# dot-comma-hyphen/oaxaca-blinder-rs

Measured on AMD Instinct MI355X. Metric: bootstrap replicates/sec on 1M-row×20-pred panel at 1/2/4/8 MI355X, higher is better.
Workload: dtype f64

## Files before the change

oaxaca-blinder-rs_amd/csrc/ob_engine.hip:

```cpp
#include <hip/hip_runtime.h>

#include <algorithm>
#include <cmath>
#include <cstdio>
#include <cstdlib>
#include <cstring>
#include <map>
#include <mutex>
#include <vector>

#include "ob_device.hpp"
#include "ob_engine.hpp"
#include "ob_hip.hpp"
#include "ob_heckman.hpp"
#include "ob_options.hpp"
#include "ob_spec.h"

typedef double ob_d4 __attribute__((ext_vector_type(4)));

namespace {

constexpr int kBlock = 256;
constexpr int kImgRow = 64;
constexpr int kImgWords = (OB_TILE_ROWS / 4) * kImgRow;
// ... 102 lines not shown
  const uint32_t c4 = c >> 12;
  ob_bitstream s = {q << 12, rep, c2, OB_TAG_L1K + rl, k0, k1, 0u, 0u, 0u, 0u, 0u};
  if (q < c4) return ky_walk(s, L, OB_KY_TABLES - 1, goff, glist);
  const uint32_t i = q - c4, nd = (uint32_t)__builtin_popcount((c >> 7) & 31u);
  if (i < nd) return ky_walk(s, L, (int)ob_l1_digit_log(c, i) - OB_KY_MIN_LOG, goff, glist);
  return ob_bs_popcount(s, c & 127u);
}

template <int DIAG>
__global__ __launch_bounds__(kBlock) __attribute__((amdgpu_waves_per_eu(8, 8))) void ob_level1_kernel(uint32_t n0, uint32_t n1, uint32_t tiles0,
                                                           uint32_t first_rep, uint32_t stride,
                                                           uint32_t key0, uint32_t key1, uint32_t* m1,
                                                           const ob_ky_tables ky_g) {
  extern __shared__ __attribute__((aligned(16))) uint32_t l1s[];
  __shared__ uint32_t s_rej, s_tail, s_acc;
  __shared__ KyLds kyl;
  const uint32_t g = blockIdx.y, rl = blockIdx.x, rep = first_rep + rl, tid = threadIdx.x;
  const uint32_t n = g ? n1 : n0;
  if (n == 0) return;
  if constexpr (!(DIAG & 4)) ky_stage(kyl, ky_g, tid);
  if constexpr ((DIAG & 16) != 0) {
    __syncthreads();
    if (tid == 0 && kyl.hlist[7] == 0xFFFFu) m1[0] = 0u;
    return;
  }
  const uint32_t T = (n + OB_TILE_ROWS - 1) >> OB_TILE_SHIFT, D = l1_depth(T), J = l1_top_levels(T);
  const uint32_t tail = n - (T - 1) * OB_TILE_ROWS;
  const bool small = l1_small(T), partial = tail < OB_TILE_ROWS;
  uint32_t* buf[2] = {l1s, l1s + l1_buf0_words(T)};
  uint32_t* top[2] = {buf[1] + (l1_sub_tiles(T) + 1) / 2, buf[1] + (l1_sub_tiles(T) + 1) / 2 + kL1TopWords};
  uint32_t* mt = l1s + 256u + 128u;
  uint32_t* mcol = m1 + (size_t)rl * stride + (g ? tiles0 : 0u);
  const uint32_t tail_owner = ((T - 1) >> 1) & (kBlock - 1);
  if (small && tid < T) mt[tid] = 0;
  uint32_t todo = n;
  for (uint32_t round = 0;; ++round) {
    if (tid == 0) {
      if (J) top[0][0] = todo;
      else buf[D & 1][0] = todo;
      s_rej = 0;
      s_tail = 0;
      s_acc = 0;
    }
    __syncthreads();
    uint32_t rej = 0;
    auto emit = [&](uint32_t t, uint32_t c) {
      if constexpr ((DIAG & 8) != 0) return;
      if (partial && t == T - 1) s_tail = c;
      else if (round == 0) mcol[t] = c;
      else if (c) mcol[t] += c;
    };
    auto level = [&](uint32_t l, uint32_t ll, uint32_t kb, uint32_t nodes, const uint32_t* cur, uint32_t* nxt) {
      const uint32_t span = 1u << (D - l - 1);
      const uint32_t nnext = (T + span - 1) / span;
      const uint32_t rl = (round << 5) + l;
      if (ll < 8) {
        const uint32_t sh = 8 - ll, k = tid >> sh, j = tid & ((1u << sh) - 1);
        if (j == 0 && k < nodes) nxt[2 * k] = 0;
        __syncthreads();
        uint32_t c = 0;
        if (k < nodes) {
          c = cur[k];
          uint32_t left = 0;
          if constexpr (DIAG & 1) left = j == 0 ? c >> 1 : 0u;
          else if (c < OB_KY_MIN_C) left = l1_split_words(j, 1u << sh, c, rep, ((kb + k) << 1) | g, rl, key0, key1);
          else
            for (uint32_t q = j, ns = ob_l1_items(c); q < ns; q += 1u << sh)
              left += l1_split_item(q, c, rep, ((kb + k) << 1) | g, rl, key0, key1, kyl, ky_g.off, ky_g.list);
          if (left) atomicAdd(&nxt[2 * k], left);
        }
        __syncthreads();
        if (j == 0 && k < nodes) {
          const uint32_t right = c - nxt[2 * k];
          if (2 * (kb + k) + 1 < nnext) nxt[2 * k + 1] = right;
          else rej += right;
        }
        __syncthreads();
      } else {
        const bool to_m1 = l + 1 == D && !small;
        for (uint32_t k = tid; k < nodes; k += kBlock) {
          const uint32_t c = cur[k], kg = kb + k;
          uint32_t left = 0;
          if constexpr (DIAG & 1) left = c >> 1;
          else if ((DIAG & 32) && c < 128u) left = c >> 1;
          else if (c < OB_KY_MIN_C) left = l1_split_words(0, 1, c, rep, (kg << 1) | g, rl, key0, key1);
          else
            for (uint32_t q = 0, ns = ob_l1_items(c); q < ns; ++q)
              left += l1_split_item(q, c, rep, (kg << 1) | g, rl, key0, key1, kyl, ky_g.off, ky_g.list);
          const uint32_t right = c - left;
          if (to_m1) {
            emit(2 * kg, left);
            if (2 * kg + 1 < T) emit(2 * kg + 1, right);
            else rej += right;
          } else {
            nxt[2 * k] = left;
            if (2 * kg + 1 < nnext) nxt[2 * k + 1] = right;
            else rej += right;
          }
        }
        __syncthreads();
      }
    };
    for (uint32_t l = 0; l < J; ++l) {
      const uint32_t span2 = 2u << (D - l - 1);
      level(l, l, 0, (T + span2 - 1) / span2, top[l & 1], top[(l + 1) & 1]);
    }
    const uint32_t nsub = J ? (T + (1u << (D - J)) - 1) >> (D - J) : 1u;
    for (uint32_t K = 0; K < nsub; ++K) {
      if (J) {
        if (tid == 0) buf[(D - J) & 1][0] = top[J & 1][K];
        __syncthreads();
      }
      for (uint32_t l = J; l < D; ++l) {
        const uint32_t ll = l - J, kb = K << ll, span2 = 2u << (D - l - 1);
        const uint32_t nodes = min(1u << ll, (T + span2 - 1) / span2 - kb);
        level(l, ll, kb, nodes, buf[(D - l) & 1], buf[(D - l - 1) & 1]);
      }
    }
    if (small) {
      const uint32_t* tl = buf[0];
      if (tid < T) {
        if (partial && tid == T - 1) s_tail = tl[tid];
        else mt[tid] += tl[tid];
      }
      __syncthreads();
    }
    if (partial && tid < 64) {
      const uint32_t c = s_tail;
      uint32_t acc = 0;
      for (uint32_t q = tid; 16 * q < c; q += 64) {
        const ob_u32x4 u = ob_philox(q, rep, g, OB_TAG_L1S + round, key0, key1);
        const uint32_t wd[4] = {u.x, u.y, u.z, u.w};
        const uint32_t m = min(16u, c - 16 * q);
#pragma unroll
        for (uint32_t i = 0; i < 16; ++i) acc += (i < m && ((wd[i >> 2] >> (8 * (i & 3))) & 0xFFu) < tail) ? 1u : 0u;
      }
      if (acc) atomicAdd(&s_acc, acc);
    }
    __syncthreads();
    if (partial) {
      const uint32_t a = s_acc;
      if (tid == 0) rej += s_tail - a;
      if (small) {
        if (tid == 0) mt[T - 1] += a;
      } else if (tid == tail_owner) {
        if (round == 0) mcol[T - 1] = a;
        else if (a) mcol[T - 1] += a;
      }
    }
    if (rej) atomicAdd(&s_rej, rej);
    __syncthreads();
    todo = s_rej;
    __syncthreads();
    if (todo <= OB_L1_DIRECT) break;
    if constexpr ((DIAG & 2) != 0) {
      todo = 0;
      break;
    }
  }
  __syncthreads();
  for (uint32_t r = tid; r < todo; r += kBlock) {
    const uint32_t thresh = (0u - n) % n;
    uint64_t x;
    for (uint32_t j = 0;; ++j) {
      const ob_u32x4 u = ob_philox(r, rep, g, OB_TAG_L1D + (j >> 2), key0, key1);
      const uint32_t wd[4] = {u.x, u.y, u.z, u.w};
      x = (uint64_t)wd[j & 3] * n;
      if ((uint32_t)x >= thresh) break;
    }
    const uint32_t t = (uint32_t)(x >> 32) >> OB_TILE_SHIFT;
    if (small) atomicAdd(&mt[t], 1u);
    else atomicAdd(&mcol[t], 1u);
  }
  if (small) {
    __syncthreads();
    if (tid < T) mcol[tid] = mt[tid];
  }
}

struct Work {
  uint32_t rb, cg, chunk, g, t0, t1, n, rep0;
  const double* X;
  int64_t ld;
};

__device__ __forceinline__ Work map_work(const GramArgs& a) {
  const uint32_t nwg = gridDim.x, bid = blockIdx.x;
  const uint32_t xcd = bid & 7u, slot = bid >> 3, q8 = nwg >> 3, r8 = nwg & 7u;
  const uint32_t wi = (xcd < r8 ? xcd * (q8 + 1) : r8 * (q8 + 1) + (xcd - r8) * q8) + slot;
  Work w;
  w.rb = wi % a.nb_rep;
  const uint32_t tq = wi / a.nb_rep;
  w.cg = tq % (uint32_t)a.n_cg;
  w.chunk = tq / (uint32_t)a.n_cg;
  w.g = a.chunks[w.chunk * 3];
  w.t0 = a.chunks[w.chunk * 3 + 1];
  w.t1 = a.chunks[w.chunk * 3 + 2];
  w.X = w.g ? a.gcols1 : a.gcols0;
  w.ld = w.g ? a.ld1 : a.ld0;
  w.n = w.g ? a.n1 : a.n0;
  w.rep0 = w.rb * 64;
  return w;
}

__device__ __forceinline__ void lds_barrier() { asm volatile("s_waitcnt lgkmcnt(0)\n\ts_barrier" ::: "memory"); }

template <int CB>
__device__ __forceinline__ void pair_offsets(const GramArgs& a, int cb0, int lane, int (&offa)[CB], int (&offb)[CB]) {
#pragma unroll
  for (int c = 0; c < CB; ++c) {
    const int e = (cb0 + c) * 16 + (lane & 15);
    int pa = 0, pb = 0;
    if (e < a.e) {
      int rem = e;
      while (rem >= a.k1 - pa) {
        rem -= a.k1 - pa;
        ++pa;
      }
      pb = pa + rem;
    }
    offa[c] = pa * kColStride + (lane >> 4) * 16 + (pa & 31);
    offb[c] = pb * kColStride + (lane >> 4) * 16 + (pb & 31);
  }
}

__device__ __forceinline__ void stage_dma(const GramArgs& a, const Work& w, uint32_t xt_byte_off, size_t gbase,
                                          int wave, int w_lo, int nw, int lane,
                                          __attribute__((address_space(3))) unsigned char* lds3) {
  const int ncl = a.k1 - a.c_first;
  const uint32_t bytes = (uint32_t)ncl * kColStride * 8;
  const char* src = reinterpret_cast<const char*>(w.X + (gbase >> 6) * (size_t)ncl * kColStride);
  const uint32_t dst = xt_byte_off + (uint32_t)a.c_first * kColStride * 8;
  for (uint32_t t = wave - w_lo; t * 1024 < bytes; t += nw)
    if (t * 1024 + lane * 16 < bytes)
      __builtin_amdgcn_global_load_lds(src + t * 1024 + lane * 16,
                                       (__attribute__((address_space(3))) void*)(lds3 + dst + t * 1024), 16, 0, 0);
}

static_assert(OB_TILE_ROWS == 256u, "full-tile draws are bytes");
__device__ __forceinline__ bool full_tile(const Work& w, uint32_t tile) {
  return w.n - tile * OB_TILE_ROWS >= OB_TILE_ROWS;
}

__device__ __forceinline__ void add_draw(uint32_t* img, uint32_t r, uint32_t lr) {
  atomicAdd(&img[(lr >> 2) * kImgRow + r], 1u << ((lr & 3u) * 8u));
}

template <int H>
__device__ __forceinline__ uint32_t sdwa_add_half(uint32_t base, uint32_t a) {
  uint32_t r;
  if constexpr (H == 0)
    asm("v_add_u32_sdwa %0, %1, %2 dst_sel:DWORD dst_unused:UNUSED_PAD src0_sel:DWORD src1_sel:WORD_0" : "=v"(r) : "v"(base), "v"(a));
  else
    asm("v_add_u32_sdwa %0, %1, %2 dst_sel:DWORD dst_unused:UNUSED_PAD src0_sel:DWORD src1_sel:WORD_1" : "=v"(r) : "v"(base), "v"(a));
  return r;
}

template <int B>
__device__ __forceinline__ uint32_t sdwa_shl_byte(uint32_t m, uint32_t one) {
  uint32_t r;
  if constexpr (B == 0)
    asm("v_lshlrev_b32_sdwa %0, %1, %2 dst_sel:DWORD dst_unused:UNUSED_PAD src0_sel:BYTE_0 src1_sel:DWORD" : "=v"(r) : "v"(m), "v"(one));
  else if constexpr (B == 1)
    asm("v_lshlrev_b32_sdwa %0, %1, %2 dst_sel:DWORD dst_unused:UNUSED_PAD src0_sel:BYTE_1 src1_sel:DWORD" : "=v"(r) : "v"(m), "v"(one));
  else if constexpr (B == 2)
    asm("v_lshlrev_b32_sdwa %0, %1, %2 dst_sel:DWORD dst_unused:UNUSED_PAD src0_sel:BYTE_2 src1_sel:DWORD" : "=v"(r) : "v"(m), "v"(one));
  else
    asm("v_lshlrev_b32_sdwa %0, %1, %2 dst_sel:DWORD dst_unused:UNUSED_PAD src0_sel:BYTE_3 src1_sel:DWORD" : "=v"(r) : "v"(m), "v"(one));
  return r;
}

template <int B>
__device__ __forceinline__ void add_draw_byte(uint32_t* img, uint32_t rep_off, uint32_t a, uint32_t m, uint32_t one) {
  atomicAdd(reinterpret_cast<uint32_t*>(reinterpret_cast<char*>(img) + sdwa_add_half<(B >> 1)>(rep_off, a)),
            sdwa_shl_byte<B>(m, one));
}

#ifndef OB_CNT_PERM
#define OB_CNT_PERM 1
#endif
template <int B>
__device__ __forceinline__ void add_draw_perm(uint32_t* img, uint32_t rep_off, uint32_t q, uint32_t m, uint32_t one) {
  const uint32_t addr = __builtin_amdgcn_perm(q, rep_off, 0x0C0C0000u | ((4u + B) << 8));
  atomicAdd(reinterpret_cast<uint32_t*>(reinterpret_cast<char*>(img) + addr), sdwa_shl_byte<B>(m, one));
}

__device__ __forceinline__ void add_draws_word(uint32_t* img, uint32_t rep_off, uint32_t w, uint32_t one) {
  const uint32_t m = (w << 3) & 0x18181818u;
  if (OB_CNT_PERM) {
    const uint32_t q = (w >> 2) & 0x3F3F3F3Fu;
    add_draw_perm<0>(img, rep_off, q, m, one);
    add_draw_perm<1>(img, rep_off, q, m, one);
    add_draw_perm<2>(img, rep_off, q, m, one);
    add_draw_perm<3>(img, rep_off, q, m, one);
    return;
  }
  const uint32_t lo = (w << 6) & 0x3F003F00u, hi = (w >> 2) & 0x3F003F00u;
  add_draw_byte<0>(img, rep_off, lo, m, one);
  add_draw_byte<1>(img, rep_off, hi, m, one);
  add_draw_byte<2>(img, rep_off, lo, m, one);
  add_draw_byte<3>(img, rep_off, hi, m, one);
}

__device__ __forceinline__ void level2_draws(const GramArgs& a, const Work& w, uint32_t tile, uint32_t* cnt,
                                             const uint32_t* mc, const uint32_t* cum, int k, int nparts, int wv,
                                             int nw, int lane) {
  const uint32_t S = min(OB_TILE_ROWS, w.n - tile * OB_TILE_ROWS);
  const bool full = S == OB_TILE_ROWS;
  const int r_lo = 64 * wv / nw, r_hi = 64 * (wv + 1) / nw, nr = r_hi - r_lo;
  if (nr <= 0) return;
  const uint32_t c_lo = cum[r_lo], C = cum[r_hi] - c_lo;
  const uint32_t f_lo = c_lo + C * (uint32_t)k / (uint32_t)nparts;
  const uint32_t f_hi = c_lo + C * (uint32_t)(k + 1) / (uint32_t)nparts;
  const uint32_t bnd = lane < nr ? cum[r_lo + 1 + lane] : 0xFFFFFFFFu;
  const uint32_t c2 = (tile << 1) | w.g;
  const uint32_t rep0 = a.first_rep + w.rep0;
  const uint32_t one = 1u;
  int rr = r_lo;
  for (uint32_t f0 = f_lo; f0 < f_hi; f0 += 64) {
    while (rr < r_hi - 1 && (uint32_t)__builtin_amdgcn_readlane(bnd, rr - r_lo) <= f0) ++rr;
    const uint32_t f = f0 + lane;
    int r = rr;
    uint32_t base = rr > r_lo ? (uint32_t)__builtin_amdgcn_readlane(bnd, rr - r_lo - 1) : c_lo;
    for (int i = rr; i < r_hi - 1; ++i) {
      const uint32_t b = (uint32_t)__builtin_amdgcn_readlane(bnd, i - r_lo);
      if (b > f0 + 63) break;
      if (f >= b) {
        r = i + 1;
        base = b;
      }
    }
    if (f < f_hi) {
      const uint32_t pp = f - base;
      ob_u32x4 u;
      if (a.diag & 64)
        u = ob_u32x4{pp * 0x9E3779B9u ^ r, pp * 0x85EBCA6Bu ^ c2, pp * 0xC2B2AE35u, pp ^ 0x27D4EB2Fu};
      else
        u = ob_philox_x3(pp, rep0 + r, c2, OB_TAG_L2, a.key0, a.key1);
      if (full && (a.diag & 32)) {
        if ((u.x ^ u.y ^ u.z ^ u.w) == 0x5EED5EEDu) cnt[r] = 1u;
      } else if (full) {
        const uint32_t wd[4] = {u.x, u.y, u.z, u.w};
#pragma unroll
        for (int i = 0; i < 4; ++i) add_draws_word(cnt, (uint32_t)r * 4u, wd[i], one);
      } else {
        add_draw(cnt, (uint32_t)r, ob_mulhi64(u.x, u.y, S));
        if (2 * pp + 1 < mc[r]) add_draw(cnt, (uint32_t)r, ob_mulhi64(u.z, u.w, S));
      }
    }
  }
  if (full && k == nparts - 1 && lane < nr) {
    const int r = r_lo + lane;
    const uint32_t m = mc[r], nd = m & 15u;
    if (nd) {
      const ob_u32x4 u = ob_philox_x3(m >> 4, rep0 + r, c2, OB_TAG_L2, a.key0, a.key1);
      const uint32_t wd[4] = {u.x, u.y, u.z, u.w};
#pragma unroll
      for (uint32_t d = 0; d < 15; ++d)
        if (d < nd) add_draw(cnt, (uint32_t)r, (wd[d >> 2] >> (8 * (d & 3))) & 0xFFu);
    }
  }
}

constexpr uint32_t kCallMapCap = 2048;

__device__ __forceinline__ void level2_map_draws(const GramArgs& a, const Work& w, uint32_t tile, uint32_t* cnt,
                                                 const uint32_t* mc, const uint32_t* cmap, uint32_t C,
                                                 uint32_t cmin, int wv, int lane) {
  const uint32_t nwin = (C + 63u) >> 6;
  const uint32_t c2 = (tile << 1) | w.g;
  const uint32_t rep0 = a.first_rep + w.rep0;
  const uint32_t one = 1u;
  for (uint32_t win = (uint32_t)wv; win <= nwin; win += 4) {
    if (win < nwin) {
      const uint32_t f = win * 64u + (uint32_t)lane;
      if (f < C) {
        uint32_t r = (uint32_t)lane, pp = win;
        if (win >= cmin) {
          const uint32_t e = cmap[f - cmin * 64u];
          r = e & 63u;
          pp = e >> 6;
        }
        ob_u32x4 u;
        if (a.diag & 64)
          u = ob_u32x4{pp * 0x9E3779B9u ^ r, pp * 0x85EBCA6Bu ^ c2, pp * 0xC2B2AE35u, pp ^ 0x27D4EB2Fu};
        else
          u = ob_philox_x3(pp, rep0 + r, c2, OB_TAG_L2, a.key0, a.key1);
        if (a.diag & 32) {
          if ((u.x ^ u.y ^ u.z ^ u.w) == 0x5EED5EEDu) cnt[r] = 1u;
        } else {
          const uint32_t wd[4] = {u.x, u.y, u.z, u.w};
#pragma unroll
          for (int i = 0; i < 4; ++i) add_draws_word(cnt, r * 4u, wd[i], one);
        }
      }
    } else {
      const uint32_t m = mc[lane], nd = m & 15u;
      if (nd) {
        const ob_u32x4 u = ob_philox_x3(m >> 4, rep0 + (uint32_t)lane, c2, OB_TAG_L2, a.key0, a.key1);
        const uint32_t wd[4] = {u.x, u.y, u.z, u.w};
#pragma unroll
        for (uint32_t d = 0; d < 15; ++d)
          if (d < nd) add_draw(cnt, (uint32_t)lane, (wd[d >> 2] >> (8 * (d & 3))) & 0xFFu);
      }
    }
  }
}

#ifndef OB_CNT_NT
#define OB_CNT_NT 0
#endif
template <bool I8>
__device__ __forceinline__ void check_store_counts(const GramArgs& a, uint32_t* cnt, uint32_t* lsum, int my,
                                                   uint32_t tt, uint32_t rb, uint32_t ns) {
  const int r = my & 63, part = my >> 6;
  uint32_t* col = cnt + part * 16 * kImgRow + r;
  uint32_t v[16];
  uint32_t sum = 0, hib = 0;
#pragma unroll
  for (int i = 0; i < 16; ++i) {
    v[i] = col[i * kImgRow];
    sum = __builtin_amdgcn_sad_u8(v[i], 0u, sum);
    hib |= v[i] & 0x80808080u;
  }
  if (I8 && hib && !(a.diag & 1632)) atomicOr(a.flags, 2u);
  if ((uint32_t)part < ns && !(a.diag & 512)) {
    if constexpr (I8) {
      uint4* out = reinterpret_cast<uint4*>(const_cast<uint32_t*>(a.counts)) + ((size_t)tt * a.nb_rep + rb) * 1024 +
                   part * 256 + (r >> 4) * 64 + (r & 15);
#pragma unroll
      for (int q = 0; q < 4; ++q) {
        if (OB_CNT_NT) {
          typedef unsigned int u32x4_t __attribute__((ext_vector_type(4)));
          const u32x4_t u4 = {v[4 * q], v[4 * q + 1], v[4 * q + 2], v[4 * q + 3]};
          __builtin_nontemporal_store(u4, reinterpret_cast<u32x4_t*>(out + q * 16));
        } else {
          out[q * 16] = make_uint4(v[4 * q], v[4 * q + 1], v[4 * q + 2], v[4 * q + 3]);
        }
      }
    } else {
      uint32_t* out = const_cast<uint32_t*>(a.counts) + ((size_t)tt * a.nb_rep + rb) * 4 * kCimgWords +
                      part * kCimgWords + r * kCimgStride;
#pragma unroll
      for (int i = 0; i < 16; ++i) out[i] = v[i];
      out[16] = 0u;
    }
  }
#pragma unroll
  for (int i = 0; i < 16; ++i) col[i * kImgRow] = 0u;
  atomicAdd(&lsum[r], sum);
}

__device__ __forceinline__ void check_sums(const GramArgs& a, uint32_t* lsum, const uint32_t* mc, int lane) {
  if (lsum[lane] != mc[lane] && !(a.diag & 1632)) atomicOr(a.flags, 1u);
  lsum[lane] = 0u;
}

__device__ __forceinline__ uint32_t level1_count(const GramArgs& a, uint32_t rep0, uint32_t tt, uint32_t r) {
  const uint32_t rep = rep0 + r;
  return rep < a.n_reps ? a.m1[(size_t)rep * a.tiles_total + tt] : 0u;
}

__device__ __forceinline__ void publish_counts(const Work& w, uint32_t tile, uint32_t m, uint32_t* mc, uint32_t* cum,
                                               int lane, uint32_t* cmap, uint32_t* cminp) {
  mc[lane] = m;
  const bool full = full_tile(w, tile);
  const uint32_t c = full ? m >> 4 : (m + 1) >> 1;
  uint32_t v = c;
#pragma unroll
  for (int o = 1; o < 64; o <<= 1) {
    const uint32_t t = __shfl_up(v, o);
    if (lane >= o) v += t;
  }
  cum[lane + 1] = v;
  if (lane == 0) cum[0] = 0;
  if (cmap && full) {
    uint32_t cmin = c, cmax = c;
#pragma unroll
    for (int o = 1; o < 64; o <<= 1) {
      cmin = min(cmin, (uint32_t)__shfl_xor(cmin, o));
      cmax = max(cmax, (uint32_t)__shfl_xor(cmax, o));
    }
    const uint32_t total = (uint32_t)__builtin_amdgcn_readlane(v, 63);
    if (total - cmin * 64u <= kCallMapCap) {
      uint32_t base = 0;
      for (uint32_t j = cmin; j < cmax; ++j) {
        const uint64_t mask = __ballot(c > j);
        if (c > j)
          cmap[base + __builtin_amdgcn_mbcnt_hi((uint32_t)(mask >> 32), __builtin_amdgcn_mbcnt_lo((uint32_t)mask, 0u))] =
              (j << 6) | (uint32_t)lane;
        base += (uint32_t)__popcll(mask);
      }
    }
    if (lane == 0) *cminp = cmin;
  }
}

template <int CB>
__device__ __forceinline__ void store_partials(const GramArgs& a, const Work& w, int cb0, int lane,
                                               const ob_d4 (&acc)[4][CB]) {
#pragma unroll
  for (int c = 0; c < CB; ++c) {
    if (cb0 + c >= a.ncb) continue;
    const int e = (cb0 + c) * 16 + (lane & 15);
#pragma unroll
    for (int q4 = 0; q4 < 4; ++q4)
#pragma unroll
      for (int r = 0; r < 4; ++r) {
        const uint32_t rep = w.rep0 + q4 * 16 + (lane >> 4) + 4 * r;
        if (rep < a.n_reps) a.partial[((size_t)w.chunk * a.rep_pad + rep) * a.e_pad + e] = acc[q4][c][r];
      }
  }
}

#ifndef OB_CNT_MAP
#define OB_CNT_MAP 1
#endif
#ifndef OB_CNT_TILES
#define OB_CNT_TILES 8
#endif
constexpr int kCntTilesPerBlock = OB_CNT_TILES;

template <bool I8>
__global__ __launch_bounds__(kBlock) void ob_count_kernel(const GramArgs a) {
  __shared__ uint32_t img[kImgWords];
  __shared__ uint32_t mcb[2][64], cumb[2][65], lsumb[2][64], cminb[2];
  __shared__ uint32_t cmap[OB_CNT_MAP ? kCallMapCap : 1];
  const int tid = threadIdx.x, lane = tid & 63, wave = tid >> 6;
  Work w{};
  w.rb = blockIdx.y;
  w.rep0 = w.rb * 64;
  const uint32_t tt0 = blockIdx.x * kCntTilesPerBlock;
  const uint32_t tt1 = min(a.tiles_total, tt0 + kCntTilesPerBlock);
  uint32_t m_next = (wave == 0 && tt0 < tt1) ? level1_count(a, w.rep0, tt0, lane) : 0u;
  for (int i = tid; i < kImgWords; i += kBlock) img[i] = 0u;
  if (tid < 128) lsumb[tid >> 6][tid & 63] = 0u;
  for (uint32_t tt = tt0; tt < tt1; ++tt) {
    uint32_t* mc = mcb[tt & 1];
    uint32_t* cum = cumb[tt & 1];
    w.g = tt >= a.tiles0 ? 1u : 0u;
    w.n = w.g ? a.n1 : a.n0;
    const uint32_t tile = tt - (w.g ? a.tiles0 : 0u);
    if (wave == 0) {
      publish_counts(w, tile, m_next, mc, cum, lane, OB_CNT_MAP ? cmap : nullptr, &cminb[tt & 1]);
      if (tt + 1 < tt1) m_next = level1_count(a, w.rep0, tt + 1, lane);
    }
    __syncthreads();
    if (wave == 0 && tt > tt0) check_sums(a, lsumb[(tt - 1) & 1], mcb[(tt - 1) & 1], lane);
    const uint32_t C = cum[64];
    const uint32_t cmin = cminb[tt & 1];
    if (a.diag & 1024) {
    } else if (OB_CNT_MAP && full_tile(w, tile) && C - cmin * 64u <= kCallMapCap)
      level2_map_draws(a, w, tile, img, mc, cmap, C, cmin, wave, lane);
    else
      level2_draws(a, w, tile, img, mc, cum, 0, 1, wave, 4, lane);
    __syncthreads();
    const uint32_t ns = (min(OB_TILE_ROWS, w.n - tile * OB_TILE_ROWS) + 63) >> 6;
    check_store_counts<I8>(a, img, lsumb[tt & 1], tid, tt, w.rb, ns);
  }
  if (tt0 < tt1) {
    __syncthreads();
    if (wave == 0) check_sums(a, lsumb[(tt1 - 1) & 1], mcb[(tt1 - 1) & 1], lane);
  }
}

constexpr int kXtOff = 2 * kCimgWords * 4;
static_assert(kXtOff % 16 == 0, "staged sub-tiles must stay 16-byte aligned");

template <int CB, bool UNIT>
__global__ __launch_bounds__(kBlock, 2) void ob_gram_kernel(const GramArgs a) {
  extern __shared__ __attribute__((aligned(16))) unsigned char smem[];
  uint32_t* cimg = reinterpret_cast<uint32_t*>(smem);
  double* xt = reinterpret_cast<double*>(smem + kXtOff);
  __attribute__((address_space(3))) unsigned char* lds3 = (__attribute__((address_space(3))) unsigned char*)smem;

  const int tid = threadIdx.x, lane = tid & 63, wave = tid >> 6;
  const Work w = map_work(a);
  const int cb0 = ((int)w.cg * 4 + wave) * CB;
  const bool mma = cb0 < a.ncb && !(a.diag & 2);
  const bool dma = !(a.diag & 4);
  const int buf_dbl = a.k1 * kColStride;
  const uint32_t tg0 = w.g ? a.tiles0 : 0u;
  auto tile_rows = [&](uint32_t t) { return min(OB_TILE_ROWS, w.n - t * OB_TILE_ROWS); };
  auto stage_counts = [&](int buf, uint32_t tile, uint32_t s) {
    if (UNIT) return;
    const uint32_t* src = a.counts + (((size_t)(tg0 + tile) * a.nb_rep + w.rb) * 4 + s) * kCimgWords;
    for (int t = wave; t * 256 < kCimgWords; t += 4)
      if (t * 256 + lane * 4 < kCimgWords)
        __builtin_amdgcn_global_load_lds(src + t * 256 + lane * 4,
                                         (__attribute__((address_space(3))) void*)(lds3 + (buf * kCimgWords + t * 256) * 4),
                                         16, 0, 0);
  };

  const bool dbl = a.dbl != 0;
  if (w.t0 < w.t1) {
    if (a.c_first == 1)
      for (int i = tid; i < kColStride; i += kBlock) {
        xt[i] = 1.0;
        if (dbl) xt[buf_dbl + i] = 1.0;
      }
    stage_dma(a, w, kXtOff, (size_t)w.t0 * OB_TILE_ROWS, wave, 0, 4, lane, lds3);
    stage_counts(0, w.t0, 0);
    asm volatile("s_waitcnt vmcnt(0)" ::: "memory");
    __syncthreads();
  }

  int offa[CB], offb[CB];
  pair_offsets<CB>(a, cb0, lane, offa, offb);
  ob_d4 acc[4][CB];
#pragma unroll
  for (int r = 0; r < 4; ++r)
#pragma unroll
    for (int c = 0; c < CB; ++c) acc[r][c] = (ob_d4){0.0, 0.0, 0.0, 0.0};
  const uint32_t sh = (uint32_t)(lane >> 4) * 8u;
  uint32_t aw[4];
  double bf[CB];
  size_t gbase = 0;
  auto read_k = [&](const uint32_t* cw, const double* xb, int ks, uint32_t (&w4)[4], double (&va)[CB],
                    double (&vb)[CB]) {
#pragma unroll
    for (int q4 = 0; q4 < 4; ++q4) w4[q4] = UNIT ? 0u : cw[q4 * 16 * kCimgStride + ks];
#pragma unroll
    for (int c = 0; c < CB; ++c) {
      va[c] = xb[offa[c] + ks];
      vb[c] = xb[offb[c] + ks];
    }
  };

  int j = 0;
  for (uint32_t tile = w.t0; tile < w.t1; ++tile) {
    const uint32_t ns = (tile_rows(tile) + 63) >> 6;
    for (uint32_t s = 0; s < ns; ++s, ++j) {
      const int cur = j & 1;
      const bool last_sub = s + 1 == ns;
      const bool has_next = !last_sub || tile + 1 < w.t1;
      const uint32_t ntile = last_sub ? tile + 1 : tile, nsub = last_sub ? 0u : s + 1;
      gbase = (size_t)tile * OB_TILE_ROWS + s * 64;
      if (has_next && dma && dbl) {
        stage_dma(a, w, kXtOff + (cur ^ 1) * buf_dbl * 8, (size_t)ntile * OB_TILE_ROWS + nsub * 64, wave, 0, 4, lane,
                  lds3);
        stage_counts(cur ^ 1, ntile, nsub);
      }
      const int cb_ = dbl ? cur : 0;
      const uint32_t* cw = cimg + cb_ * kCimgWords + (lane & 15) * kCimgStride;
      const double* xb = xt + cb_ * buf_dbl;
      if (mma) {
        {
          double va[CB], vb[CB];
          read_k(cw, xb, 0, aw, va, vb);
#pragma unroll
          for (int c = 0; c < CB; ++c) bf[c] = va[c] * vb[c];
        }
#pragma unroll
        for (int ks = 0; ks < 16; ++ks) {
          uint32_t an[4];
          double na[CB], nb[CB];
          if (ks < 15) read_k(cw, xb, ks + 1, an, na, nb);
          __builtin_amdgcn_sched_barrier(0);
          double af[4];
#pragma unroll
          for (int q4 = 0; q4 < 4; ++q4)
            af[q4] = UNIT ? ((gbase + ks * 4 + (lane >> 4) < w.n) ? 1.0 : 0.0) : (double)((aw[q4] >> sh) & 0xFFu);
#pragma unroll
          for (int q4 = 0; q4 < 4; ++q4)
#pragma unroll
            for (int c = 0; c < CB; ++c)
              acc[q4][c] = __builtin_amdgcn_mfma_f64_16x16x4f64(af[q4], bf[c], acc[q4][c], 0, 0, 0);
          __builtin_amdgcn_sched_barrier(0);
          if (ks < 15) {
#pragma unroll
            for (int q4 = 0; q4 < 4; ++q4) aw[q4] = an[q4];
#pragma unroll
            for (int c = 0; c < CB; ++c) bf[c] = na[c] * nb[c];
          }
          __builtin_amdgcn_sched_barrier(0);
        }
      }
      if (!dbl && has_next && dma) {
        lds_barrier();
        stage_dma(a, w, kXtOff, (size_t)ntile * OB_TILE_ROWS + nsub * 64, wave, 0, 4, lane, lds3);
        stage_counts(0, ntile, nsub);
      }
      asm volatile("s_waitcnt vmcnt(0)" ::: "memory");
      lds_barrier();
    }
  }
  if (mma) store_partials<CB>(a, w, cb0, lane, acc);
}

__global__ __launch_bounds__(kBlock) void ob_reduce_kernel(const double* partial, const uint32_t* chunks,
                                                           int n_chunks, uint32_t rep_pad, int e_pad,
                                                           uint32_t n_reps, double* gram) {
  const size_t i = (size_t)blockIdx.x * kBlock + threadIdx.x;
  if (i >= (size_t)n_reps * e_pad) return;
  const uint32_t rep = (uint32_t)(i / e_pad);
  const int e = (int)(i % e_pad);
  double s0 = 0.0, s1 = 0.0;
  for (int c = 0; c < n_chunks; ++c) {
    const double v = partial[((size_t)c * rep_pad + rep) * e_pad + e];
    if (chunks[c * 3] == 0)
      s0 += v;
    else
      s1 += v;
  }
  gram[((size_t)rep * 2 + 0) * e_pad + e] = s0;
  gram[((size_t)rep * 2 + 1) * e_pad + e] = s1;
}

struct SolveArgs {
  const double* gram;
  int e_pad, k1, k, pool_pos, ref_mode, weighted;
  int yc;
  double rows_a, rows_b;
  int n_norm, n_base;
  const int32_t* norm;
  int off_idx, off_m, off_pstart, off_pidx, off_has;
  double* rows;
  uint8_t* ok;
  int row_len;
  uint32_t n_reps;
  double* gram_out;
  double* raw_beta_b;
  int raw_status;
};

__device__ void normalize_coeffs(double* beta, const SolveArgs& a, const int32_t* starts,
                                 const int32_t* idx, double* base) {
  for (int v = 0; v < a.n_norm; ++v) {
    const int s = starts[v], e = starts[v + 1];
    base[v] = 0.0;
    if (e == s) continue;
    double sum = 0.0;
    for (int t = s; t < e; ++t) sum += beta[idx[t]];
    const int cat = a.norm[a.off_m + v];
    const int mm = cat >= 0 ? cat : (e - s) + 1;
    if (mm == 0) continue;
    const double mean = sum / (double)mm;
    base[v] = -mean;
    beta[0] += mean;
    for (int t = s; t < e; ++t) beta[idx[t]] -= mean;
  }
}

template <bool DUAL>
__global__ __launch_bounds__(128) void ob_solve_kernel(const SolveArgs a) {
  extern __shared__ __attribute__((aligned(16))) double sm[];
  __shared__ int st_sh[2];
  const int lane = threadIdx.x & 63, w = DUAL ? (int)(threadIdx.x >> 6) : 0;
  const uint32_t rep = blockIdx.x;
  if (rep >= a.n_reps) return;
  const int k = a.k, k1 = a.k1, kp = k + 1;
  double* M = sm;
  double* M1 = M + kp * kp;
  double* rhs = M1 + (DUAL ? k * k : 0);
  double* rhs1 = rhs + kp;
  double* beta_a = rhs1 + kp;
  double* beta_b = beta_a + kp;
  double* xam = beta_b + kp;
  double* xbm = xam + kp;
  double* bstar = xbm + kp;
  double* base = bstar + kp;
  const double* GA = a.gram + (size_t)rep * 2 * a.e_pad;
  const double* GB = GA + a.e_pad;
  double* row = a.rows + (size_t)rep * a.row_len;
  if (a.gram_out && rep == 0)
    for (int i = threadIdx.x; i < 2 * a.e_pad; i += blockDim.x) a.gram_out[i] = GA[i];

  int ok_g = 1;
  for (int g = w; g < 2; g += DUAL ? 2 : 1) {
    const double* G = g ? GB : GA;
    double* beta = g ? beta_b : beta_a;
    double* Mg = (DUAL && g) ? M1 : M;
    double* rg = (DUAL && g) ? rhs1 : rhs;
    for (int i = lane; i < k * k; i += 64) {
      const int r = i % k, c = i / k;
      Mg[r + c * k] = gpair(G, r, c, k1);
    }
    for (int i = lane; i < k; i += 64) rg[i] = gpair(G, i, a.yc, k1);
    ob_sync<DUAL>();
    if (!wave_cholesky<DUAL>(Mg, k, lane)) {
      ok_g = 0;
      break;
    }
    wave_chol_solve<DUAL>(Mg, k, rg, lane);
    if (g == 1 && a.raw_beta_b && rep == 0)
      for (int i = lane; i < k; i += 64) a.raw_beta_b[i] = rg[i];
    const double sw = G[0];
    for (int i = lane; i < k; i += 64) {
      beta[i] = rg[i];
      (g ? xbm : xam)[i] = gpair(G, 0, i, k1) / sw;
    }
  }
  if (lane == 0) st_sh[w] = ok_g;
  __syncthreads();
  if (w != 0) return;
  uint8_t status = (st_sh[0] && (!DUAL || st_sh[1])) ? 1 : 0;
  const int32_t* nst = a.norm;
  const int32_t* nidx = a.norm + a.off_idx;
  const int32_t* pst = a.norm + a.off_pstart;
  const int32_t* pidx = a.norm + a.off_pidx;
  const int32_t* has = a.norm + a.off_has;
  double* base_a = base;
  double* base_b = base + a.n_norm;
  double* base_s = base + 2 * a.n_norm;
  if (status == 1 && a.n_norm > 0) {
    if (lane == 0) {
      normalize_coeffs(beta_a, a, nst, nidx, base_a);
      normalize_coeffs(beta_b, a, nst, nidx, base_b);
      for (int v = 0; v < a.n_norm; ++v) base_s[v] = 0.0;
    }
    ob_sync<DUAL>();
  }
  if (status == 1) {
    if (a.ref_mode == OB_REF_GROUP_A || a.ref_mode == OB_REF_GROUP_B) {
      const double* src = a.ref_mode == OB_REF_GROUP_A ? beta_a : beta_b;
      for (int i = lane; i < k; i += 64) bstar[i] = src[i];
      if (lane == 0)
        for (int v = 0; v < a.n_norm; ++v) base_s[v] = a.ref_mode == OB_REF_GROUP_A ? base_a[v] : base_b[v];
    } else if (a.ref_mode == OB_REF_WEIGHTED || a.ref_mode == OB_REF_COTTON) {
      const double sa = a.weighted ? GA[0] : a.rows_a;
      const double sb = a.weighted ? GB[0] : a.rows_b;
      const double tot = sa + sb;
      if (tot == 0.0) {
        status = 2;
      } else {
        const double wA = sa / tot, wB = 1.0 - wA;
        for (int i = lane; i < k; i += 64) bstar[i] = beta_a[i] * wA + beta_b[i] * wB;
        if (lane == 0)
          for (int v = 0; v < a.n_norm; ++v) base_s[v] = base_a[v] * wA + base_b[v] * wB;
      }
    } else {
      const int ip = a.pool_pos;
      for (int i = lane; i < kp * kp; i += 64) {
        const int u = i % kp, v = i / kp;
        double val;
        if (u == ip && v == ip) {
          val = GA[0];
        } else if (u == ip || v == ip) {
          const int o = (u == ip) ? (v < ip ? v : v - 1) : (u < ip ? u : u - 1);
          val = gpair(GA, 0, o, k1);
        } else {
          const int ou = u < ip ? u : u - 1, ov = v < ip ? v : v - 1;
          val = gpair(GA, ou, ov, k1) + gpair(GB, ou, ov, k1);
        }
        M[u + v * kp] = val;
      }
      for (int u = lane; u < kp; u += 64) {
        if (u == ip) {
          rhs[u] = gpair(GA, 0, a.yc, k1);
        } else {
          const int o = u < ip ? u : u - 1;
          rhs[u] = gpair(GA, o, a.yc, k1) + gpair(GB, o, a.yc, k1);
        }
      }
      ob_sync<DUAL>();
      if (!wave_cholesky<DUAL>(M, kp, lane)) {
        status = 0;
      } else {
        wave_chol_solve<DUAL>(M, kp, rhs, lane);
        if (lane == 0) {
          if (a.n_norm > 0) normalize_coeffs(rhs, a, pst, pidx, base_s);
          for (int u = 0, d = 0; u < kp; ++u)
            if (u != ip) bstar[d++] = rhs[u];
        }
      }
    }
// ... 1248 lines not shown
```

Before: 693,100.

## Overlap next-tile count publishing with draws and use DPP wave scans

Restructures the count kernel so the next tile's level-1 counts are loaded and published by the least-loaded wave while the current tile's draws run. The call map becomes double-buffered, and the publish/sync step before each tile's draws is dropped in favour of a barrier after the store. Prefix-sum and min/max reductions switch from shuffle loops to DPP row operations, and the partial-call tail draws reuse the word/byte packed adders instead of per-draw calls. The call-map cap is halved, which means fewer tiles qualify for the mapped path and shared memory stays within budget, at the cost of an extra barrier per tile.

```diff
diff --git a/oaxaca-blinder-rs_amd/csrc/ob_engine.hip b/oaxaca-blinder-rs_amd/csrc/ob_engine.hip
--- a/oaxaca-blinder-rs_amd/csrc/ob_engine.hip
+++ b/oaxaca-blinder-rs_amd/csrc/ob_engine.hip
@@ -428,6 +428,31 @@
   add_draw_byte<3>(img, rep_off, hi, m, one);
 }
 
+__device__ __forceinline__ void add_draws_bytes(uint32_t* img, uint32_t rep_off, uint32_t w, uint32_t one, uint32_t n) {
+  const uint32_t m = (w << 3) & 0x18181818u;
+  if (OB_CNT_PERM) {
+    const uint32_t q = (w >> 2) & 0x3F3F3F3Fu;
+    if (n > 0) add_draw_perm<0>(img, rep_off, q, m, one);
+    if (n > 1) add_draw_perm<1>(img, rep_off, q, m, one);
+    if (n > 2) add_draw_perm<2>(img, rep_off, q, m, one);
+    return;
+  }
+  const uint32_t lo = (w << 6) & 0x3F003F00u, hi = (w >> 2) & 0x3F003F00u;
+  if (n > 0) add_draw_byte<0>(img, rep_off, lo, m, one);
+  if (n > 1) add_draw_byte<1>(img, rep_off, hi, m, one);
+  if (n > 2) add_draw_byte<2>(img, rep_off, lo, m, one);
+}
+
+__device__ __forceinline__ void part_call_draws(uint32_t* img, uint32_t r, uint32_t nd, const ob_u32x4& u,
+                                                uint32_t one) {
+  const uint32_t nw = nd >> 2;
+  if (nw > 0) add_draws_word(img, r * 4u, u.x, one);
+  if (nw > 1) add_draws_word(img, r * 4u, u.y, one);
+  if (nw > 2) add_draws_word(img, r * 4u, u.z, one);
+  const uint32_t wl = nw == 0 ? u.x : nw == 1 ? u.y : nw == 2 ? u.z : u.w;
+  add_draws_bytes(img, r * 4u, wl, one, nd & 3u);
+}
+
 __device__ __forceinline__ void level2_draws(const GramArgs& a, const Work& w, uint32_t tile, uint32_t* cnt,
                                              const uint32_t* mc, const uint32_t* cum, int k, int nparts, int wv,
                                              int nw, int lane) {
@@ -480,15 +505,12 @@
     const uint32_t m = mc[r], nd = m & 15u;
     if (nd) {
       const ob_u32x4 u = ob_philox_x3(m >> 4, rep0 + r, c2, OB_TAG_L2, a.key0, a.key1);
-      const uint32_t wd[4] = {u.x, u.y, u.z, u.w};
-#pragma unroll
-      for (uint32_t d = 0; d < 15; ++d)
-        if (d < nd) add_draw(cnt, (uint32_t)r, (wd[d >> 2] >> (8 * (d & 3))) & 0xFFu);
-    }
-  }
-}
-
-constexpr uint32_t kCallMapCap = 2048;
+      part_call_draws(cnt, (uint32_t)r, nd, u, one);
+    }
+  }
+}
+
+constexpr uint32_t kCallMapCap = 1024;
 
 __device__ __forceinline__ void level2_map_draws(const GramArgs& a, const Work& w, uint32_t tile, uint32_t* cnt,
                                                  const uint32_t* mc, const uint32_t* cmap, uint32_t C,
@@ -524,10 +546,7 @@
       const uint32_t m = mc[lane], nd = m & 15u;
       if (nd) {
         const ob_u32x4 u = ob_philox_x3(m >> 4, rep0 + (uint32_t)lane, c2, OB_TAG_L2, a.key0, a.key1);
-        const uint32_t wd[4] = {u.x, u.y, u.z, u.w};
-#pragma unroll
-        for (uint32_t d = 0; d < 15; ++d)
-          if (d < nd) add_draw(cnt, (uint32_t)lane, (wd[d >> 2] >> (8 * (d & 3))) & 0xFFu);
+        part_call_draws(cnt, (uint32_t)lane, nd, u, one);
       }
     }
   }
@@ -587,26 +606,34 @@
   return rep < a.n_reps ? a.m1[(size_t)rep * a.tiles_total + tt] : 0u;
 }
 
+template <int CTRL, int ROWS>
+__device__ __forceinline__ uint32_t dpp_take(uint32_t v, uint32_t idle) {
+  return (uint32_t)__builtin_amdgcn_update_dpp((int)idle, (int)v, CTRL, ROWS, 0xF, false);
+}
+template <class Op>
+__device__ __forceinline__ uint32_t wave_scan(uint32_t v, uint32_t idle, Op op) {
+  v = op(v, dpp_take<0x111, 0xF>(v, idle));
+  v = op(v, dpp_take<0x112, 0xF>(v, idle));
+  v = op(v, dpp_take<0x114, 0xF>(v, idle));
+  v = op(v, dpp_take<0x118, 0xF>(v, idle));
+  v = op(v, dpp_take<0x142, 0xA>(v, idle));
+  v = op(v, dpp_take<0x143, 0xC>(v, idle));
+  return v;
+}
+
 __device__ __forceinline__ void publish_counts(const Work& w, uint32_t tile, uint32_t m, uint32_t* mc, uint32_t* cum,
                                                int lane, uint32_t* cmap, uint32_t* cminp) {
   mc[lane] = m;
   const bool full = full_tile(w, tile);
   const uint32_t c = full ? m >> 4 : (m + 1) >> 1;
-  uint32_t v = c;
-#pragma unroll
-  for (int o = 1; o < 64; o <<= 1) {
-    const uint32_t t = __shfl_up(v, o);
-    if (lane >= o) v += t;
-  }
+  const uint32_t v = wave_scan(c, 0u, [](uint32_t x, uint32_t y) { return x + y; });
   cum[lane + 1] = v;
   if (lane == 0) cum[0] = 0;
   if (cmap && full) {
-    uint32_t cmin = c, cmax = c;
-#pragma unroll
-    for (int o = 1; o < 64; o <<= 1) {
-      cmin = min(cmin, (uint32_t)__shfl_xor(cmin, o));
-      cmax = max(cmax, (uint32_t)__shfl_xor(cmax, o));
-    }
+    const uint32_t cmin = (uint32_t)__builtin_amdgcn_readlane(
+        wave_scan(c, 0xFFFFFFFFu, [](uint32_t x, uint32_t y) { return min(x, y); }), 63);
+    const uint32_t cmax =
+        (uint32_t)__builtin_amdgcn_readlane(wave_scan(c, 0u, [](uint32_t x, uint32_t y) { return max(x, y); }), 63);
     const uint32_t total = (uint32_t)__builtin_amdgcn_readlane(v, 63);
     if (total - cmin * 64u <= kCallMapCap) {
       uint32_t base = 0;
@@ -651,43 +678,55 @@
 __global__ __launch_bounds__(kBlock) void ob_count_kernel(const GramArgs a) {
   __shared__ uint32_t img[kImgWords];
   __shared__ uint32_t mcb[2][64], cumb[2][65], lsumb[2][64], cminb[2];
-  __shared__ uint32_t cmap[OB_CNT_MAP ? kCallMapCap : 1];
+  __shared__ uint32_t cmapb[2][kCallMapCap];
   const int tid = threadIdx.x, lane = tid & 63, wave = tid >> 6;
   Work w{};
   w.rb = blockIdx.y;
   w.rep0 = w.rb * 64;
   const uint32_t tt0 = blockIdx.x * kCntTilesPerBlock;
   const uint32_t tt1 = min(a.tiles_total, tt0 + kCntTilesPerBlock);
-  uint32_t m_next = (wave == 0 && tt0 < tt1) ? level1_count(a, w.rep0, tt0, lane) : 0u;
+  if (tt0 >= tt1) return;
   for (int i = tid; i < kImgWords; i += kBlock) img[i] = 0u;
   if (tid < 128) lsumb[tid >> 6][tid & 63] = 0u;
+  if (wave == 0) {
+    w.g = tt0 >= a.tiles0 ? 1u : 0u;
+    w.n = w.g ? a.n1 : a.n0;
+    publish_counts(w, tt0 - (w.g ? a.tiles0 : 0u), level1_count(a, w.rep0, tt0, lane), mcb[tt0 & 1], cumb[tt0 & 1], lane,
+                   cmapb[tt0 & 1], &cminb[tt0 & 1]);
+  }
+  __syncthreads();
   for (uint32_t tt = tt0; tt < tt1; ++tt) {
-    uint32_t* mc = mcb[tt & 1];
-    uint32_t* cum = cumb[tt & 1];
+    const uint32_t* mc = mcb[tt & 1];
     w.g = tt >= a.tiles0 ? 1u : 0u;
     w.n = w.g ? a.n1 : a.n0;
     const uint32_t tile = tt - (w.g ? a.tiles0 : 0u);
-    if (wave == 0) {
-      publish_counts(w, tile, m_next, mc, cum, lane, OB_CNT_MAP ? cmap : nullptr, &cminb[tt & 1]);
-      if (tt + 1 < tt1) m_next = level1_count(a, w.rep0, tt + 1, lane);
-    }
-    __syncthreads();
-    if (wave == 0 && tt > tt0) check_sums(a, lsumb[(tt - 1) & 1], mcb[(tt - 1) & 1], lane);
-    const uint32_t C = cum[64];
+    const uint32_t C = cumb[tt & 1][64];
     const uint32_t cmin = cminb[tt & 1];
+    const bool mapped = OB_CNT_MAP && full_tile(w, tile) && C - cmin * 64u <= kCallMapCap;
+    const bool pub = (uint32_t)wave == (mapped ? (((C + 63u) >> 6) + 1u) & 3u : 0u);
+    uint32_t m_next = 0u;
+    if (pub && tt + 1 < tt1) m_next = level1_count(a, w.rep0, tt + 1, lane);
     if (a.diag & 1024) {
-    } else if (OB_CNT_MAP && full_tile(w, tile) && C - cmin * 64u <= kCallMapCap)
-      level2_map_draws(a, w, tile, img, mc, cmap, C, cmin, wave, lane);
+    } else if (mapped)
+      level2_map_draws(a, w, tile, img, mc, cmapb[tt & 1], C, cmin, wave, lane);
     else
-      level2_draws(a, w, tile, img, mc, cum, 0, 1, wave, 4, lane);
+      level2_draws(a, w, tile, img, mc, cumb[tt & 1], 0, 1, wave, 4, lane);
+    if (pub) {
+      if (tt > tt0) check_sums(a, lsumb[(tt - 1) & 1], mcb[(tt - 1) & 1], lane);
+      if (tt + 1 < tt1) {
+        Work wn = w;
+        wn.g = tt + 1 >= a.tiles0 ? 1u : 0u;
+        wn.n = wn.g ? a.n1 : a.n0;
+        publish_counts(wn, tt + 1 - (wn.g ? a.tiles0 : 0u), m_next, mcb[(tt + 1) & 1], cumb[(tt + 1) & 1], lane,
+                       cmapb[(tt + 1) & 1], &cminb[(tt + 1) & 1]);
+      }
+    }
     __syncthreads();
     const uint32_t ns = (min(OB_TILE_ROWS, w.n - tile * OB_TILE_ROWS) + 63) >> 6;
     check_store_counts<I8>(a, img, lsumb[tt & 1], tid, tt, w.rb, ns);
-  }
-  if (tt0 < tt1) {
     __syncthreads();
-    if (wave == 0) check_sums(a, lsumb[(tt1 - 1) & 1], mcb[(tt1 - 1) & 1], lane);
-  }
+  }
+  if (wave == 0) check_sums(a, lsumb[(tt1 - 1) & 1], mcb[(tt1 - 1) & 1], lane);
 }
 
 constexpr int kXtOff = 2 * kCimgWords * 4;
```

Result: faster. 703,100 (median of 6 runs) (+1.4%).
